# Bai-YT/ConsistencyTTA

Measured on AMD Instinct MI355X. Metric: 10s_audio_clips_per_sec_1step_gen, higher is better.
Workload: dtype bf16; 1 GPU; configs[1]: batch-32 single-step consistency inference, U-Net(light, 559M) + AudioLDM VAE decoder + HiFi-GAN, 10 s clips, L=32 text tokens, w=4, T5 excluded; batch_per_gpu=32, global_batch=32, text_len=32, waveform_samples=163872, weights=random-init (no checkpoints offline), parallelism=replicas x1 (clips sharded, no data-path collective)

## Files before the change

consistencytta_amd/_native.py:

```python
import ctypes
from ctypes import byref
import os
import subprocess
from ctypes import (POINTER, Structure, c_char_p, c_double, c_float, c_int, c_int16, c_int32,
                    c_int64, c_size_t, c_uint8, c_void_p)

_HERE = os.path.dirname(os.path.abspath(__file__))
LIB_PATH = os.path.join(_HERE, "libctta_hip.so")
CSRC = os.path.join(_HERE, "csrc")

MAX_LEVELS = 4
MAX_UPS = 8


class Tensor(Structure):
    _fields_ = [("name", c_char_p), ("data", c_void_p), ("ndim", c_int), ("shape", c_int64 * 4)]


class UNetConfig(Structure):
    _fields_ = [
        ("in_channels", c_int), ("out_channels", c_int), ("n_levels", c_int),
        ("block_out_channels", c_int * MAX_LEVELS), ("heads", c_int * MAX_LEVELS),
        ("layers_per_block", c_int * MAX_LEVELS), ("down_cross", c_int * MAX_LEVELS),
        ("up_cross", c_int * MAX_LEVELS), ("cross_attention_dim", c_int),
# ... 26 lines not shown
        ("n_kernels", c_int), ("upsample_rates", c_int * MAX_UPS),
        ("upsample_kernel_sizes", c_int * MAX_UPS), ("resblock_kernel_sizes", c_int * 4),
        ("resblock_dilations", (c_int * 3) * 4), ("max_batch", c_int), ("max_frames", c_int),
        ("debug_taps", c_int), ("enable_grad", c_int),
    ]


class FfnDesc(Structure):
    _fields_ = [("x", c_void_p), ("ld_x", c_int), ("M", c_int64), ("cp", c_int), ("ffp", c_int),
                ("packed", c_void_p), ("b1", c_void_p), ("b2", c_void_p), ("res", c_void_p), ("res_ld", c_int),
                ("out", c_void_p), ("ldc", c_int), ("n_valid", c_int),
                ("ln_gamma", c_void_p), ("ln_beta", c_void_p), ("ln_d", c_int), ("ln_eps", c_float),
                ("proj_packed", c_void_p), ("proj_bias", c_void_p), ("proj_res", c_void_p), ("proj_res_ld", c_int),
                ("front_packed", c_void_p), ("front_bias", c_void_p), ("att", c_void_p), ("att_ld", c_int), ("front_k", c_int),
                ("front_res", c_void_p), ("front_res_ld", c_int), ("s2_out", c_void_p), ("s2_ld", c_int)]


class ConvDesc(Structure):
    _fields_ = [
        ("x0", c_void_p), ("c0", c_int), ("x1", c_void_p), ("c1", c_int),
        ("batch", c_int), ("hi", c_int), ("wi", c_int), ("upsample", c_int),
        ("ho", c_int), ("wo", c_int),
        ("kh", c_int), ("kw", c_int), ("stride_h", c_int), ("stride_w", c_int),
        ("pad_h", c_int), ("pad_w", c_int), ("dil_h", c_int), ("dil_w", c_int),
        ("w", c_void_p), ("k_pad", c_int), ("n", c_int),
        ("bias", c_void_p), ("bias_m", c_void_p), ("rowvec", c_void_p), ("rowvec_ld", c_int),
        ("res", c_void_p), ("res_ld", c_int),
        ("in_act", c_int), ("in_slope", c_float), ("out_act", c_int), ("out_slope", c_float),
        ("alpha", c_float), ("accumulate", c_int), ("out", c_void_p), ("ldc", c_int), ("out_f32", c_int),
        ("out2", c_void_p), ("out2_slope", c_float),
# ... 136 lines not shown
    "ctta_wav_to_logmel_db_bwd": (c_int, [c_void_p, c_void_p, c_int, c_int, c_float, c_void_p, c_void_p]),
    "ctta_htsat_image": (c_int, [c_void_p, c_int, c_int, c_int, c_void_p, c_void_p, c_void_p, c_void_p, c_int, c_int, c_int,
                                 c_void_p, c_void_p]),
    "ctta_htsat_image_bwd": (c_int, [c_void_p, c_int, c_int, c_int, c_int, c_int, c_void_p, c_void_p, c_void_p, c_void_p,
                                     c_int, c_void_p, c_void_p]),
    "ctta_gather_rows": (c_int, [c_void_p, c_int, c_void_p, c_void_p, c_int, c_int64, c_int, c_void_p]),
    "ctta_gelu": (c_int, [c_void_p, c_void_p, c_int64, c_void_p]),
    "ctta_gelu_bwd": (c_int, [c_void_p, c_void_p, c_void_p, c_int64, c_void_p]),
    "ctta_mean_tokens": (c_int, [c_void_p, c_int, c_int, c_int, c_int, c_void_p, c_void_p]),
    "ctta_mean_tokens_bwd": (c_int, [c_void_p, c_int, c_int, c_int, c_int, c_void_p, c_void_p]),
    "ctta_resunit_supported": (c_int, [c_int, c_int, c_int]),
    "ctta_ffn_desc_init": (None, [c_void_p]),
    "ctta_ffn_proj_pack_bytes": (c_size_t, [c_int, c_int]),
    "ctta_ffn_proj_pack": (c_int, [c_void_p, c_int, c_int, c_int, c_void_p, c_void_p]),
    "ctta_ffn_block": (c_int, [c_void_p, c_void_p]),
    "ctta_ffn_geglu_supported": (c_int, [c_int, c_int]),
    "ctta_ffn_geglu_wanted": (c_int, [c_int, c_int, c_int64]),
    "ctta_ffn_pack_bytes": (c_size_t, [c_int, c_int]),
    "ctta_ffn_pack": (c_int, [c_void_p, c_int, c_void_p, c_int, c_int, c_int, c_void_p, c_void_p]),
    "ctta_ffn_geglu": (c_int, [c_void_p, c_int, c_int64, c_int, c_int, c_void_p, c_void_p, c_void_p, c_void_p, c_int, c_void_p,
                               c_int, c_int, c_void_p, c_void_p, c_int, c_float, c_void_p]),
    "ctta_frag_pack": (c_int, [c_void_p, c_int, c_int, c_int, c_void_p, c_void_p]),
    "ctta_resunit_conv1d": (c_int, [c_void_p, c_int, c_int, c_int, c_int, c_int, c_void_p, c_void_p, c_void_p, c_void_p,
                                    c_float, c_void_p, c_int, c_float, c_float, c_void_p]),
    "ctta_logmel_to_image": (c_int, [c_void_p, c_int, c_int, c_int, c_void_p, c_void_p, c_void_p, c_void_p]),
    "ctta_avgpool2": (c_int, [c_void_p, c_void_p, c_int, c_int, c_int, c_int, c_void_p]),
    "ctta_cnn14_head": (c_int, [c_void_p, c_int, c_int, c_int, c_int, c_void_p, c_void_p]),
    "ctta_reschain_supported": (c_int, [c_int, c_int, c_void_p]),
    "ctta_reschain_conv1d": (c_int, [c_void_p, c_int, c_int, c_int, c_int, c_void_p, c_void_p, c_void_p, c_void_p, c_void_p,
                                     c_float, c_void_p, c_int, c_float, c_float, c_void_p]),
# ... 143 lines not shown
```

consistencytta_amd/csrc/common.h:

```cpp
#pragma once
#include <hip/hip_runtime.h>
#include <stdint.h>
#include <stdio.h>
#include <string.h>

#include "../../include/ctta.h"

typedef uint16_t bf16_t;

typedef __attribute__((ext_vector_type(8))) __bf16 bf16x8_t;
typedef __attribute__((ext_vector_type(4))) float f32x4_t;

__device__ __forceinline__ float bf2f(bf16_t v) { return __uint_as_float(((uint32_t)v) << 16); }

typedef __attribute__((ext_vector_type(2))) __bf16 bf16x2_t;
typedef __attribute__((ext_vector_type(2))) float f32x2_t;
__device__ __forceinline__ bf16_t f2bf(float f) { return __builtin_bit_cast(bf16_t, (__bf16)f); }

__device__ __forceinline__ uint32_t pack2bf(float lo, float hi) {
  const f32x2_t v = {lo, hi};
  return __builtin_bit_cast(uint32_t, __builtin_convertvector(v, bf16x2_t));
}

__device__ __forceinline__ void unpack8(const uint4& v, float f[8]) {
// ... 48 lines not shown
template <int GL>
__device__ __forceinline__ float ln_group_sum(float v) {
  v = dpp_row_sum(v);
  {
    const unsigned u = __float_as_uint(v);
    const auto r = __builtin_amdgcn_permlane16_swap(u, u, false, false);
    v = __uint_as_float(r[0]) + __uint_as_float(r[1]);
  }
  if constexpr (GL == 64) {
    const unsigned u = __float_as_uint(v);
    const auto r = __builtin_amdgcn_permlane32_swap(u, u, false, false);
    v = __uint_as_float(r[0]) + __uint_as_float(r[1]);
  }
  return v;
}
__device__ __forceinline__ float wave_sum(float v) {
#pragma unroll
  for (int o = 32; o > 0; o >>= 1) v += __shfl_xor(v, o, 64);
  return v;
}
__device__ __forceinline__ float wave_max(float v) {
#pragma unroll
  for (int o = 32; o > 0; o >>= 1) v = fmaxf(v, __shfl_xor(v, o, 64));
  return v;
}

enum CttaOption {
  CTTA_OPT_XCD = 0,
  CTTA_OPT_SPLITK,
  CTTA_OPT_STREAMK,
  CTTA_OPT_STREAMK_GRID,
  CTTA_OPT_WGRAD_STREAM,
  CTTA_OPT_GN_FUSE,
  CTTA_OPT_FUSED_RES,
  CTTA_OPT_FFN_FUSE,
  CTTA_OPT_COUNT
};
extern int g_ctta_opt[CTTA_OPT_COUNT];
int ctta_cu_count();
static inline int ctta_opt(CttaOption o) { return g_ctta_opt[o]; }
void ctta_set_error(const char* fmt, ...);
bool ctta_prof_active();
bool ctta_gn_fuse_on();
unsigned long long* ctta_debug_stamps_current();
void ctta_prof_begin(int kind, int variant, long long m, long long n, long long k, long long groups, hipStream_t s);
void ctta_prof_end(hipStream_t s);
hipError_t ctta_zero_async(void* ptr, size_t bytes, hipStream_t s);

#define CTTA_CHECK_HIP(expr)                                                         \
  do {                                                                               \
    hipError_t _e = (expr);                                                          \
    if (_e != hipSuccess) {                                                          \
      ctta_set_error("%s:%d: %s -> %s", __FILE__, __LINE__, #expr, hipGetErrorString(_e)); \
      return CTTA_ERR_HIP;                                                           \
    }                                                                                \
  } while (0)

#define CTTA_REQUIRE(cond, ...)                \
// ... 26 lines not shown
```

consistencytta_amd/csrc/engine_unet.hip:

```cpp
#include "engine_common.h"

#include <stdlib.h>

#include <math.h>

__global__ void add_silu_kernel(const float* __restrict__ a, const float* __restrict__ b,
                                float* __restrict__ out, float* __restrict__ sum_out, int n) {
  const int i = blockIdx.x * blockDim.x + threadIdx.x;
  if (i >= n) return;
  const float v = a[i] + (b ? b[i] : 0.f);
  if (sum_out) sum_out[i] = v;
  out[i] = v / (1.0f + expf(-v));
}
__global__ void mask_bias_kernel(const uint8_t* __restrict__ m, float* __restrict__ out, int n) {
  const int i = blockIdx.x * blockDim.x + threadIdx.x;
  if (i < n) out[i] = (1.0f - (m[i] ? 1.0f : 0.0f)) * -10000.0f;
}
__global__ void pack_enc_kernel(const float* __restrict__ src, bf16_t* __restrict__ dst, int B, int L,
                                int X, int Lp, int Xp) {
  const long long total = (long long)B * Lp * Xp;
  for (long long i = blockIdx.x * (long long)blockDim.x + threadIdx.x; i < total;
       i += (long long)gridDim.x * blockDim.x) {
    const int x = (int)(i % Xp);
    const long long r = i / Xp;
// ... 26 lines not shown
  struct Saved { const bf16_t *x = nullptr, *a = nullptr, *t1 = nullptr, *a2 = nullptr; float *st1 = nullptr, *st2 = nullptr; int H = 0, W = 0; } sv;
};

struct LNLayer { float* gamma = nullptr; float* beta = nullptr; std::string key; };

struct Transformer {
  int c = 0, heads = 0, dh = 0, inner = 0, cp = 0, hp = 0, ffh = 0, ffp = 0;
  GNLayer norm;
  PackedW proj_in, qk1, v1, out1, q2, k2, v2, out2, ff1, ff2, proj_out;
  LNLayer ln1, ln2, ln3;
  bf16_t *k2c = nullptr, *vt2c = nullptr;
  bf16_t* ffn_stream = nullptr;
  bool want_proj_stream = false;
  bf16_t* front_stream = nullptr;
  bf16_t* proj_stream = nullptr;
  LinTrain t_proj_in, t_q1, t_k1, t_v1, t_out1, t_q2, t_k2, t_v2, t_out2, t_ff1, t_ff2, t_proj_out;
  struct Saved {
    const bf16_t *x = nullptr, *g = nullptr, *s0 = nullptr, *n1 = nullptr, *qk = nullptr, *vt = nullptr, *att1 = nullptr,
                 *s1 = nullptr, *n2 = nullptr, *q2 = nullptr, *k2 = nullptr, *vt2 = nullptr, *att2 = nullptr, *s2 = nullptr,
                 *n3 = nullptr, *f = nullptr, *gg = nullptr, *s3 = nullptr;
    float *st = nullptr, *lse1 = nullptr, *lse2 = nullptr;
    int H = 0, W = 0;
  } sv;
};

struct Level {
  std::vector<Resnet> res;
  std::vector<Transformer> att;
  bool has_sampler = false;
  ConvLayer sampler;
// ... 162 lines not shown
    ws.jobs.push_back([=](const WeightTable&, hipStream_t s) -> ctta_status { return ctta_ffn_pack(w1, k1, w2, k2, cp, ffp, dst, s); });
    T->want_proj_stream = true;
  }
  CTTA_TRY(make_ln(ws, t + "norm1.", inner, &T->ln1));
  CTTA_TRY(make_ln(ws, t + "norm2.", inner, &T->ln2));
  CTTA_TRY(make_ln(ws, t + "norm3.", inner, &T->ln3));
  CTTA_TRY(lin(p + "proj_out.weight", p + "proj_out.bias", c, inner, identity_map(c, round_up(c, 4)), in_cols,
               &T->proj_out, &T->t_proj_out));
  if (T->want_proj_stream && T->out2.n == cp && T->out2.k_pad == hp && T->out2.bias && ctta_ffn_proj_pack_bytes(cp, hp)) {
    T->front_stream = reinterpret_cast<bf16_t*>(ws.arena.get<unsigned char>(ctta_ffn_proj_pack_bytes(cp, hp)));
    if (!T->front_stream) { ctta_set_error("weight store exhausted (front projection weight stream)"); return CTTA_ERR_NOMEM; }
    const bf16_t* w0 = T->out2.w;
    bf16_t* dst = T->front_stream;
    ws.jobs.push_back([=](const WeightTable&, hipStream_t s) -> ctta_status { return ctta_ffn_proj_pack(w0, hp, hp, cp, dst, s); });
  }
  if (T->want_proj_stream && T->proj_out.n == cp && T->proj_out.k_pad == cp && c == cp) {
    T->proj_stream = reinterpret_cast<bf16_t*>(ws.arena.get<unsigned char>(ctta_ffn_proj_pack_bytes(cp, cp)));
    if (!T->proj_stream) { ctta_set_error("weight store exhausted (projection weight stream)"); return CTTA_ERR_NOMEM; }
    const bf16_t* w3 = T->proj_out.w;
    bf16_t* dst = T->proj_stream;
    ws.jobs.push_back([=](const WeightTable&, hipStream_t s) -> ctta_status { return ctta_ffn_proj_pack(w3, cp, cp, cp, dst, s); });
  }
  return CTTA_OK;
}

static ctta_status gn(UCtx& c, const GNLayer& g, const bf16_t* x, bf16_t* y, int hw, float eps, bool silu,
                      float** stats_out = nullptr) {
  const int groups = c.U->cfg.norm_num_groups;
  size_t need = ctta_groupnorm_scratch_floats(c.B, hw, g.c, groups);
  if (c.train) {
// ... 43 lines not shown
  }
  RUN(c, ctta_attention_lse(q, q_ld, k, k_ld, k_rows, vt, vt_ld, bias, out, out_ld, c.B, heads, nq, nk,
                            1.0f / sqrtf((float)dh), lse, c.stream));
  return CTTA_OK;
}

static ctta_status run_transformer(UCtx& c, Transformer& T, const bf16_t* x, int H, int W,
                                   bf16_t** out_p) {
  Arena& A = *c.arena;
  const int N = H * W;
  const size_t M = (size_t)c.B * N;
  const int cp = T.cp, hp = T.hp;
  bf16_t* out = A.get<bf16_t>(M * T.c); ALLOC_OR_FAIL(out);
  const size_t mk = A.mark();
  bf16_t* g = A.get<bf16_t>(M * T.c); ALLOC_OR_FAIL(g);
  CTTA_TRY(gn(c, T.norm, x, g, N, 1e-6f, false, &T.sv.st));
  bf16_t* s0 = A.get<bf16_t>(M * cp); ALLOC_OR_FAIL(s0);
  CTTA_TRY(run_linear(c, T.proj_in, g, T.c, M, s0, cp, nullptr, 0));
  bf16_t* n = A.get<bf16_t>(M * cp); ALLOC_OR_FAIL(n);
  RUN(c, ctta_layernorm(s0, n, M, T.inner, cp, T.ln1.gamma, T.ln1.beta, 1e-5f, c.stream));
  bf16_t* qk = A.get<bf16_t>(M * 2 * hp); ALLOC_OR_FAIL(qk);
  CTTA_TRY(run_linear(c, T.qk1, n, cp, M, qk, 2 * hp, nullptr, 0));
  const int vt_ld = round_up(N, 8);
  bf16_t* vt = A.get<bf16_t>((size_t)c.B * hp * vt_ld); ALLOC_OR_FAIL(vt);
  CTTA_TRY(run_vt(c, T.v1, n, c.B, N, N, vt, vt_ld));
  bf16_t* att = A.get<bf16_t>(M * hp); ALLOC_OR_FAIL(att);
  CTTA_TRY(run_attention(c, qk, 2 * hp, qk + hp, 2 * hp, N, vt, vt_ld, nullptr, att, hp, T.heads, N, N, T.dh, &T.sv.lse1));
  bf16_t* s1 = A.get<bf16_t>(M * cp); ALLOC_OR_FAIL(s1);
  CTTA_TRY(run_linear(c, T.out1, att, hp, M, s1, cp, s0, cp));
  bf16_t* const n1 = n;
  bf16_t* const att1 = att;
  if (c.train) {
    n = A.get<bf16_t>(M * cp); ALLOC_OR_FAIL(n);
    att = A.get<bf16_t>(M * hp); ALLOC_OR_FAIL(att);
  }
  RUN(c, ctta_layernorm(s1, n, M, T.inner, cp, T.ln2.gamma, T.ln2.beta, 1e-5f, c.stream));
  bf16_t* const n2 = n;
  bf16_t* q2 = A.get<bf16_t>(M * hp); ALLOC_OR_FAIL(q2);
  CTTA_TRY(run_linear(c, T.q2, n, cp, M, q2, hp, nullptr, 0));
  bf16_t* k2 = T.k2c;
  bf16_t* vt2 = T.vt2c;
  if (!k2 || c.dry) {
    k2 = A.get<bf16_t>((size_t)c.B * c.Lp * hp); ALLOC_OR_FAIL(k2);
    vt2 = A.get<bf16_t>((size_t)c.B * hp * c.Lp); ALLOC_OR_FAIL(vt2);
  }
  if (!c.reuse_text) {
    CTTA_TRY(run_linear(c, T.k2, c.enc_bf, c.U->xp, (int64_t)c.B * c.Lp, k2, hp, nullptr, 0));
    CTTA_TRY(run_vt(c, T.v2, c.enc_bf, c.B, c.Lp, c.Lp, vt2, c.Lp));
  }
  CTTA_TRY(run_attention(c, q2, hp, k2, hp, c.Lp, vt2, c.Lp, c.mask_bias, att, hp, T.heads, N, c.L, T.dh, &T.sv.lse2));
  bf16_t* s2 = A.get<bf16_t>(M * cp); ALLOC_OR_FAIL(s2);
  const bool ffn_fused = !c.train && T.ffn_stream && ctta_ffn_geglu_wanted(cp, T.ffp, (int64_t)M);
  const bool ffn_front = ffn_fused && T.front_stream;
  if (!ffn_front) {
    CTTA_TRY(run_linear(c, T.out2, att, hp, M, s2, cp, s1, cp));
    if (c.train) { n = A.get<bf16_t>(M * cp); ALLOC_OR_FAIL(n); }
    RUN(c, ctta_layernorm(s2, n, M, T.inner, cp, T.ln3.gamma, T.ln3.beta, 1e-5f, c.stream));
  }
  bf16_t* f = nullptr;
  bf16_t* gg = nullptr;
  if (c.train) {
    f = A.get<bf16_t>(M * 2 * T.ffp); ALLOC_OR_FAIL(f);
    CTTA_TRY(run_linear(c, T.ff1, n, cp, M, f, 2 * T.ffp, nullptr, 0));
    gg = A.get<bf16_t>(M * T.ffp); ALLOC_OR_FAIL(gg);
    RUN(c, ctta_geglu(f, gg, M, T.ffp, 1, c.stream));
  } else if (ffn_fused) {
    ctta_ffn_desc fd;
// ... 550 lines not shown
```

consistencytta_amd/csrc/norm_elem.hip:

```cpp
#include "common.h"

#include <math.h>
#include <stdlib.h>

__global__ void nchw_to_nhwc_kernel(const float* __restrict__ src, bf16_t* __restrict__ dst, int B,
                                    int C, int HW, int Cp, float scale) {
  const int vc = Cp / 8;
  const long long total = (long long)B * HW * vc;
  for (long long idx = blockIdx.x * (long long)blockDim.x + threadIdx.x; idx < total;
       idx += (long long)gridDim.x * blockDim.x) {
    const int v = (int)(idx % vc);
    const long long pix = idx / vc;
    const int b = (int)(pix / HW);
    const int hw = (int)(pix - (long long)b * HW);
    float f[8];
#pragma unroll
    for (int e = 0; e < 8; ++e) {
      const int c = v * 8 + e;
      f[e] = c < C ? src[((size_t)b * C + c) * HW + hw] * scale : 0.f;
    }
    *reinterpret_cast<uint4*>(dst + (size_t)pix * Cp + v * 8) = pack8(f);
  }
}

// ... 259 lines not shown
  __syncthreads();
  const int cpg = C / G;
  for (int g = tid; g < G; g += 256) {
    float s = 0.f, q = 0.f;
    for (int l = 0; l < PL; ++l)
      for (int cc = 0; cc < cpg; ++cc) {
        s += ssum[l * C + g * cpg + cc];
        q += ssq[l * C + g * cpg + cc];
      }
    float* o = part + (((size_t)b * nchunk + chunk) * G + g) * 2;
    o[0] = s;
    o[1] = q;
  }
}

__device__ __forceinline__ void gn_fold_chunks(const float* __restrict__ pg, int nchunk, int G, int l, int LPG, double& s,
                                               double& q) {
  constexpr int U = 8;
  for (int ch = l; ch < nchunk; ch += LPG * U) {
    float2 pp[U];
#pragma unroll
    for (int u = 0; u < U; ++u) {
      const int c = ch + u * LPG;
      pp[u] = c < nchunk ? *reinterpret_cast<const float2*>(pg + (size_t)c * G * 2) : make_float2(0.f, 0.f);
    }
#pragma unroll
    for (int u = 0; u < U; ++u) {
      s += (double)pp[u].x;
      q += (double)pp[u].y;
    }
  }
}

__global__ __launch_bounds__(256) void gn_finalize_kernel(const float* __restrict__ part, int nchunk, int G, int C,
                                                          int HW, const float* __restrict__ gamma,
                                                          const float* __restrict__ beta, float eps,
                                                          float* __restrict__ scale_shift, float* __restrict__ stats) {
  const int b = blockIdx.x;
  const int cpg = C / G;
  int LPG = 1;
  if (G <= 128 && 256 % G == 0) LPG = min(64, 256 / G);
  const int per_pass = 256 / LPG;
  for (int g0 = 0; g0 < G; g0 += per_pass) {
    const int g = g0 + (int)threadIdx.x / LPG, l = (int)threadIdx.x % LPG;
    double s = 0.0, q = 0.0;
    if (g < G) gn_fold_chunks(part + ((size_t)b * nchunk * G + g) * 2, nchunk, G, l, LPG, s, q);
    for (int off = 1; off < LPG; off <<= 1) {
// ... 828 lines not shown
```

include/ctta.h:

```cpp
#ifndef CTTA_H
#define CTTA_H

#include <stddef.h>
#include <stdint.h>

#ifdef __cplusplus
extern "C" {
#endif

typedef enum {
  CTTA_OK = 0,
  CTTA_ERR_INVALID = 1,
  CTTA_ERR_HIP = 2,
  CTTA_ERR_MISSING_KEY = 3,
  CTTA_ERR_NOMEM = 4
} ctta_status;

const char* ctta_last_error(void);
int ctta_version(void);

ctta_status ctta_set_option(const char* name, int value);
ctta_status ctta_get_option(const char* name, int* value);
int ctta_num_options(void);
const char* ctta_option_name(int i);
// ... 214 lines not shown
  int x_stride;
  void* gn_part; int gn_groups; int gn_hw;
  int64_t gn_part_floats;
} ctta_conv_desc;

ctta_status ctta_conv_gemm(const ctta_conv_desc* d, void* stream);
int ctta_conv_last_gn_chunks(void);
void ctta_conv_bind_workspace(void* ws, size_t bytes);
void ctta_conv_bind_workspace_ex(void* ws, size_t bytes, int header_zeroed);
int ctta_conv_bound_workspace_header(void);
size_t ctta_conv_workspace_header_bytes(void);
void ctta_conv_bound_workspace(void** ws, size_t* bytes);
void ctta_conv_suppress_splitk(int on);
void ctta_conv_debug_stamps(void* buf);
void ctta_attention_debug_stamps(void* buf);
size_t ctta_conv_workspace_bytes(void);
int ctta_conv_gemm_num_variants(void);
const char* ctta_conv_gemm_variant_name(int id);

int ctta_resunit_supported(int channels, int k, int dil);
ctta_status ctta_frag_pack(const void* packed, int n, int k_pad, int k_valid, void* dst, void* stream);
ctta_status ctta_resunit_conv1d(const void* x, int batch, int len, int channels, int k, int dil,
                                const void* w1_frag, const float* b1, const void* w2_frag, const float* b2,
                                float slope, void* out, int accumulate, float alpha, float out_slope, void* stream);
int ctta_reschain_supported(int channels, int k, const int* dils);
ctta_status ctta_reschain_conv1d(const void* x, int batch, int len, int channels, int k, const int* dils,
                                 const void* const* w1_frag, const float* const* b1, const void* const* w2_frag,
                                 const float* const* b2, float slope, void* out, int accumulate, float alpha,
                                 float out_slope, void* stream);

// ... 7 lines not shown
                           const float* ln_gamma, const float* ln_beta, int ln_d, float ln_eps, void* stream);
typedef struct {
  const void* x; int ld_x; int64_t M; int cp, ffp;
  const void* packed; const float* b1; const float* b2;
  const void* res; int res_ld;
  void* out; int ldc; int n_valid;
  const float* ln_gamma; const float* ln_beta; int ln_d; float ln_eps;
  const void* proj_packed; const float* proj_bias; const void* proj_res; int proj_res_ld;
  const void* front_packed; const float* front_bias; const void* att; int att_ld; int front_k;
  const void* front_res; int front_res_ld; void* s2_out; int s2_ld;
} ctta_ffn_desc;
void ctta_ffn_desc_init(ctta_ffn_desc* d);
size_t ctta_ffn_proj_pack_bytes(int cp, int k);
ctta_status ctta_ffn_proj_pack(const void* w_packed, int k_pad, int k, int cp, void* dst, void* stream);
ctta_status ctta_ffn_block(const ctta_ffn_desc* d, void* stream);

ctta_status ctta_conv_small_n(const void* x, int c, int batch, int hi, int wi, int kh, int kw,
                              int pad_h, int pad_w, const float* w, const float* bias, int n,
                              int in_act, float in_slope, int out_act, float* out_nchw,
                              void* out_bf16_nhwc, void* stream);

ctta_status ctta_pack_weight(const float* src, const int32_t* row_off, const int32_t* col_off,
                             const int32_t* row_aux, const int32_t* col_aux, int aux_limit,
                             int n_rows, int k_pad, void* dst, void* stream);

#define CTTA_PACK_ELEMS_PER_BLOCK 2048
#define CTTA_COPY_ELEMS_PER_BLOCK 16384
typedef struct {
  const float* src;
  const int32_t *row_off, *col_off, *row_aux, *col_aux;
// ... 218 lines not shown
```

Measured before the change: 436.3 clips/s.

## Fuse GroupNorm, proj_in, LayerNorm and QKV projections into one attention-head kernel

Adds a single kernel that finalizes GroupNorm statistics from the existing partial sums and applies GN to a row tile held in shared memory. The same kernel then runs proj_in with bias (also writing s0), applies LayerNorm in place, and computes the QK projection and the transposed V projection from weights prepacked per wave. It replaces a GN launch, two linear layers, a layernorm and a V-transpose GEMM, cutting launches and global round trips of intermediates. It only engages for cp 256/512 when the tile grid fills the device and GN partials are ready; otherwise the old path runs. Costs are extra packed-weight memory and a large hand-written kernel.

```diff
diff --git a/consistencytta_amd/_native.py b/consistencytta_amd/_native.py
--- a/consistencytta_amd/_native.py
+++ b/consistencytta_amd/_native.py
@@ -64,6 +64,14 @@
                 ("proj_packed", c_void_p), ("proj_bias", c_void_p), ("proj_res", c_void_p), ("proj_res_ld", c_int),
                 ("front_packed", c_void_p), ("front_bias", c_void_p), ("att", c_void_p), ("att_ld", c_int), ("front_k", c_int),
                 ("front_res", c_void_p), ("front_res_ld", c_int), ("s2_out", c_void_p), ("s2_ld", c_int)]
+
+
+class AttnHeadDesc(Structure):
+    _fields_ = [("x", c_void_p), ("x_ld", c_int), ("batch", c_int), ("tokens", c_int), ("c", c_int), ("cp", c_int), ("hp", c_int),
+                ("rows", c_int), ("gn_table", c_void_p), ("gn_partials", c_void_p), ("gn_nchunk", c_int), ("gn_groups", c_int),
+                ("gn_gamma", c_void_p), ("gn_beta", c_void_p), ("gn_eps", c_float), ("packed", c_void_p), ("b_in", c_void_p),
+                ("s0", c_void_p), ("s0_ld", c_int), ("ln_gamma", c_void_p), ("ln_beta", c_void_p), ("ln_d", c_int),
+                ("ln_eps", c_float), ("qk", c_void_p), ("qk_ld", c_int), ("vt", c_void_p), ("vt_ld", c_int)]
 
 
 class ConvDesc(Structure):
@@ -230,6 +238,13 @@
     "ctta_ffn_proj_pack_bytes": (c_size_t, [c_int, c_int]),
     "ctta_ffn_proj_pack": (c_int, [c_void_p, c_int, c_int, c_int, c_void_p, c_void_p]),
     "ctta_ffn_block": (c_int, [c_void_p, c_void_p]),
+    "ctta_attn_chain_debug_mode": (None, [c_int]),
+    "ctta_attn_head_desc_init": (None, [c_void_p]),
+    "ctta_attn_head_supported": (c_int, [c_int, c_int, c_int, c_int]),
+    "ctta_attn_head_wanted": (c_int, [c_int, c_int, c_int, c_int]),
+    "ctta_attn_head_pack_bytes": (c_size_t, [c_int, c_int]),
+    "ctta_attn_head_pack": (c_int, [c_void_p, c_int, c_void_p, c_int, c_void_p, c_int, c_int, c_int, c_void_p, c_void_p]),
+    "ctta_attn_head_chain": (c_int, [c_void_p, c_void_p]),
     "ctta_ffn_geglu_supported": (c_int, [c_int, c_int]),
     "ctta_ffn_geglu_wanted": (c_int, [c_int, c_int, c_int64]),
     "ctta_ffn_pack_bytes": (c_size_t, [c_int, c_int]),
diff --git a/consistencytta_amd/csrc/attn_chain.hip b/consistencytta_amd/csrc/attn_chain.hip
--- /dev/null
+++ b/consistencytta_amd/csrc/attn_chain.hip
@@ -0,0 +1,404 @@
+#include "conv_epilogue.h"
+
+#include <string.h>
+
+#include <type_traits>
+
+typedef unsigned u32x2_t __attribute__((ext_vector_type(2)));
+typedef unsigned u32x4_t __attribute__((ext_vector_type(4)));
+
+#ifndef CTTA_ATTN_CHAIN
+#define CTTA_ATTN_CHAIN 1
+#endif
+
+constexpr int AC_NW = 8;
+constexpr int AC_PF = 2;
+constexpr int HEAD_ROWS_256 = 128, HEAD_ROWS_512 = 64;
+
+struct HeadParams {
+  const bf16_t* x; int x_ld;
+  const float* table;
+  const float* part; int nchunk, G;
+  const float* gn_gamma; const float* gn_beta; float gn_eps;
+  int tokens;
+  const bf16_t* win; const float* bin;
+  bf16_t* s0; int s0_ld;
+  const float* ln_gamma; const float* ln_beta; int ln_d; float ln_eps;
+  const bf16_t* wqk; bf16_t* qk; int qk_ld;
+  const bf16_t* wv; bf16_t* vt; int vt_ld, hp;
+  int M, batch;
+};
+
+template <int NC, int PB>
+__device__ __forceinline__ void ac_gemm(const uint4* wp, const bf16_t* base, const int rs, const int steps, const int lq, const int lg,
+                                        f32x4_t (&acc)[NC][PB]) {
+  constexpr int PF = NC > 2 ? 1 : AC_PF;
+  bf16x8_t r0[PF + 1][NC];
+#pragma unroll
+  for (int i = 0; i < NC; ++i)
+#pragma unroll
+    for (int j = 0; j < PB; ++j) acc[i][j] = (f32x4_t){0.f, 0.f, 0.f, 0.f};
+#pragma unroll
+  for (int s = 0; s < PF; ++s)
+#pragma unroll
+    for (int i = 0; i < NC; ++i) r0[s][i] = __builtin_bit_cast(bf16x8_t, wp[(s * NC + i) * 64]);
+  wp += PF * NC * 64;
+  const bf16_t* bw = base + lq * rs + lg * 8;
+  for (int st = 0; st < steps; ++st) {
+#pragma unroll
+    for (int i = 0; i < NC; ++i) r0[PF][i] = __builtin_bit_cast(bf16x8_t, wp[(st * NC + i) * 64]);
+    __builtin_amdgcn_sched_barrier(0);
+#pragma unroll
+    for (int pb = 0; pb < PB; ++pb) {
+      const bf16x8_t bf = __builtin_bit_cast(bf16x8_t, *reinterpret_cast<const uint4*>(bw + pb * 16 * rs + st * 32));
+#pragma unroll
+      for (int i = 0; i < NC; ++i) acc[i][pb] = __builtin_amdgcn_mfma_f32_16x16x32_bf16(r0[0][i], bf, acc[i][pb], 0, 0, 0);
+    }
+#pragma unroll
+    for (int s = 0; s < PF; ++s)
+#pragma unroll
+      for (int i = 0; i < NC; ++i) r0[s][i] = r0[s + 1][i];
+  }
+}
+
+template <int CP, int BM>
+__device__ __forceinline__ void ac_layernorm_tile(bf16_t* atile, const int tid, const float* __restrict__ gamma, const float* __restrict__ beta,
+                                                  const int d, const float eps) {
+  constexpr int RS = CP + 8, CV = CP / 8, RPS = 512 / CV, NSW = BM / RPS;
+  const int cc = tid % CV, rr = tid / CV;
+  const float inv_d = 1.0f / (float)d;
+  float g[8], bt[8];
+#pragma unroll
+  for (int e = 0; e < 8; ++e) {
+    const int c = cc * 8 + e;
+    g[e] = c < d ? gamma[c] : 0.f;
+    bt[e] = c < d ? beta[c] : 0.f;
+  }
+#pragma unroll
+  for (int u = 0; u < NSW; ++u) {
+    float f[8];
+    unpack8(*reinterpret_cast<const uint4*>(atile + (rr + u * RPS) * RS + cc * 8), f);
+    float sum = 0.f;
+#pragma unroll
+    for (int e = 0; e < 8; ++e) {
+      if (cc * 8 + e >= d) f[e] = 0.f;
+      sum += f[e];
+    }
+    const float mean = ln_group_sum<CV>(sum) * inv_d;
+    float q = 0.f;
+#pragma unroll
+    for (int e = 0; e < 8; ++e)
+      if (cc * 8 + e < d) { const float t = f[e] - mean; q += t * t; }
+    const float rstd = rsqrtf(ln_group_sum<CV>(q) * inv_d + eps);
+    float o8[8];
+#pragma unroll
+    for (int e = 0; e < 8; ++e) o8[e] = cc * 8 + e < d ? (f[e] - mean) * rstd * g[e] + bt[e] : 0.f;
+    *reinterpret_cast<uint4*>(atile + (rr + u * RPS) * RS + cc * 8) = pack8(o8);
+  }
+}
+
+template <int S, int PB, bool VT>
+__device__ __forceinline__ void ac_col_passes(const uint4* wq, const bf16_t* tile, const int rs, bf16_t* out, const int ldc, const int n_out,
+                                              const size_t out_bytes, const int row0_off, const int w, const int lane) {
+  const int lq = lane & 15, lg = lane >> 4;
+  const __amdgpu_buffer_rsrc_t rso = __builtin_amdgcn_make_buffer_rsrc((void*)out, 0, (unsigned)out_bytes, 0x00020000);
+  const int ngroups = (n_out + 127) / 128;
+  auto pass = [&](auto nc_tag, const int col) {
+    constexpr int NC = decltype(nc_tag)::value;
+    const uint4* wp = wq + (size_t)w * (S + AC_PF) * NC * 64 + lane;
+    bf16x8_t r0[AC_PF + 1][NC];
+    f32x4_t acc[NC][PB];
+#pragma unroll
+    for (int i = 0; i < NC; ++i)
+#pragma unroll
+      for (int j = 0; j < PB; ++j) acc[i][j] = (f32x4_t){0.f, 0.f, 0.f, 0.f};
+#pragma unroll
+    for (int s = 0; s < AC_PF; ++s)
+#pragma unroll
+      for (int i = 0; i < NC; ++i) r0[s][i] = __builtin_bit_cast(bf16x8_t, wp[(s * NC + i) * 64]);
+    wp += AC_PF * NC * 64;
+    const bf16_t* bw = tile + lq * rs + lg * 8;
+#pragma unroll
+    for (int st = 0; st < S; ++st) {
+#pragma unroll
+      for (int i = 0; i < NC; ++i) r0[AC_PF][i] = __builtin_bit_cast(bf16x8_t, wp[(st * NC + i) * 64]);
+      __builtin_amdgcn_sched_barrier(0);
+#pragma unroll
+      for (int pb = 0; pb < PB; ++pb) {
+        const bf16x8_t bf = __builtin_bit_cast(bf16x8_t, *reinterpret_cast<const uint4*>(bw + pb * 16 * rs + st * 32));
+#pragma unroll
+        for (int i = 0; i < NC; ++i)
+          acc[i][pb] = VT ? __builtin_amdgcn_mfma_f32_16x16x32_bf16(bf, r0[0][i], acc[i][pb], 0, 0, 0)
+                          : __builtin_amdgcn_mfma_f32_16x16x32_bf16(r0[0][i], bf, acc[i][pb], 0, 0, 0);
+      }
+#pragma unroll
+      for (int s = 0; s < AC_PF; ++s)
+#pragma unroll
+        for (int i = 0; i < NC; ++i) r0[s][i] = r0[s + 1][i];
+    }
+#pragma unroll
+    for (int i = 0; i < NC; ++i) {
+      const int blk = col + (w * NC + i) * 16;
+      const bool live = blk < n_out;
+      const int vo = !live ? (int)0x80000000 : VT ? row0_off + ((blk + lq) * ldc + lg * 4) * 2 : row0_off + (lq * ldc + blk + lg * 4) * 2;
+#pragma unroll
+      for (int pb = 0; pb < PB; ++pb) {
+        const f32x4_t a = acc[i][pb];
+        u32x2_t pk;
+        pk[0] = pack2bf(a[0], a[1]);
+        pk[1] = pack2bf(a[2], a[3]);
+        __builtin_amdgcn_raw_buffer_store_b64(pk, rso, vo + (VT ? pb * 16 * 2 : pb * 16 * ldc * 2), 0, 0);
+      }
+    }
+  };
+  int col = 0;
+  for (int gp = 0; gp + 2 <= ngroups; gp += 2) {
+    pass(std::integral_constant<int, 2>{}, col);
+    wq += (size_t)AC_NW * (S + AC_PF) * 2 * 64;
+    col += 256;
+  }
+  if (ngroups & 1) pass(std::integral_constant<int, 1>{}, col);
+}
+
+
+template <int CP, int BM>
+__global__ __launch_bounds__(512, 4) void attn_head_kernel(const HeadParams p) {
+  constexpr int RS = CP + 8, S1 = CP / 32, NC2 = CP / 16 / AC_NW, PB = BM / 16;
+  constexpr int CV = CP / 8, RPS = 512 / CV, NSW = BM / RPS;
+  extern __shared__ __attribute__((aligned(16))) unsigned char smem_raw[];
+  bf16_t* atile = reinterpret_cast<bf16_t*>(smem_raw);
+  float* ss = reinterpret_cast<float*>(smem_raw + (size_t)BM * RS * 2);
+  const int tid = threadIdx.x, lane = tid & 63, w = __builtin_amdgcn_readfirstlane(tid >> 6);
+  const int lq = lane & 15, lg = lane >> 4;
+  const int m0 = blockIdx.x * BM, b = m0 / p.tokens;
+
+  {
+    const int cc = tid % CV, rr = tid / CV;
+    const __amdgpu_buffer_rsrc_t rsx =
+        __builtin_amdgcn_make_buffer_rsrc((void*)p.x, 0, (unsigned)((size_t)p.M * p.x_ld * 2), 0x00020000);
+    u32x4_t v[NSW];
+#pragma unroll
+    for (int u = 0; u < NSW; ++u) v[u] = __builtin_amdgcn_raw_buffer_load_b128(rsx, ((m0 + rr + u * RPS) * p.x_ld + cc * 8) * 2, 0, 0);
+    const float* tab = p.table ? p.table + (size_t)b * 2 * CP : ss;
+    if (!p.table) {
+      if (tid < 256) {
+        const int G = p.G, nchunk = p.nchunk, cpg = CP / G;
+        int LPG = 1;
+        if (G <= 128 && 256 % G == 0) LPG = min(64, 256 / G);
+        const int per_pass = 256 / LPG;
+        for (int g0 = 0; g0 < G; g0 += per_pass) {
+          const int g = g0 + tid / LPG, l = tid % LPG;
+          double s = 0.0, q = 0.0;
+          if (g < G) gn_fold_chunks(p.part + ((size_t)b * nchunk * G + g) * 2, nchunk, G, l, LPG, s, q);
+          for (int off = 1; off < LPG; off <<= 1) {
+            s += __shfl_xor(s, off);
+            q += __shfl_xor(q, off);
+          }
+          if (g >= G) continue;
+          const double n = (double)p.tokens * cpg;
+          const double mean = s / n;
+          double var = q / n - mean * mean;
+          if (var < 0.0) var = 0.0;
+          const float rstd = (float)(1.0 / sqrt(var + (double)p.gn_eps));
+          const float meanf = (float)mean;
+          for (int c2 = l; c2 < cpg; c2 += LPG) {
+            const int c = g * cpg + c2;
+            const float sc = rstd * p.gn_gamma[c];
+            ss[c] = sc;
+            ss[CP + c] = p.gn_beta[c] - meanf * sc;
+          }
+        }
+      }
+      __syncthreads();
+    }
+    float scl[8], shf[8];
+#pragma unroll
+    for (int e = 0; e < 8; ++e) { scl[e] = tab[cc * 8 + e]; shf[e] = tab[CP + cc * 8 + e]; }
+#pragma unroll
+    for (int u = 0; u < NSW; ++u) {
+      float f[8];
+      unpack8(make_uint4(v[u][0], v[u][1], v[u][2], v[u][3]), f);
+#pragma unroll
+      for (int e = 0; e < 8; ++e) f[e] = f[e] * scl[e] + shf[e];
+      *reinterpret_cast<uint4*>(atile + (rr + u * RPS) * RS + cc * 8) = pack8(f);
+    }
+  }
+  __syncthreads();
+
+  {
+    f32x4_t acc[NC2][PB];
+    ac_gemm<NC2, PB>(reinterpret_cast<const uint4*>(p.win) + (size_t)w * (S1 + AC_PF) * NC2 * 64 + lane, atile, RS, S1, lq, lg, acc);
+    __syncthreads();
+    const __amdgpu_buffer_rsrc_t rso =
+        __builtin_amdgcn_make_buffer_rsrc((void*)p.s0, 0, (unsigned)((size_t)p.M * p.s0_ld * 2), 0x00020000);
+    const int n0 = w * NC2 * 16 + lg * 4;
+#pragma unroll
+    for (int i = 0; i < NC2; ++i) {
+      const int n = n0 + i * 16;
+      const float4 bb = *reinterpret_cast<const float4*>(p.bin + n);
+      const int vo = ((m0 + lq) * p.s0_ld + n) * 2;
+#pragma unroll
+      for (int pb = 0; pb < PB; ++pb) {
+        const f32x4_t a = acc[i][pb];
+        u32x2_t pk;
+        pk[0] = pack2bf(a[0] + bb.x, a[1] + bb.y);
+        pk[1] = pack2bf(a[2] + bb.z, a[3] + bb.w);
+        *reinterpret_cast<u32x2_t*>(atile + (pb * 16 + lq) * RS + n) = pk;
+        __builtin_amdgcn_raw_buffer_store_b64(pk, rso, vo + pb * 16 * p.s0_ld * 2, 0, 0);
+      }
+    }
+  }
+  __syncthreads();
+
+  ac_layernorm_tile<CP, BM>(atile, tid, p.ln_gamma, p.ln_beta, p.ln_d, p.ln_eps);
+  __syncthreads();
+
+  ac_col_passes<S1, PB, false>(reinterpret_cast<const uint4*>(p.wqk), atile, RS, p.qk, p.qk_ld, 2 * p.hp, (size_t)p.M * p.qk_ld * 2,
+                               m0 * p.qk_ld * 2, w, lane);
+  ac_col_passes<S1, PB, true>(reinterpret_cast<const uint4*>(p.wv), atile, RS, p.vt, p.vt_ld, p.hp, (size_t)p.batch * p.hp * p.vt_ld * 2,
+                              (b * p.hp * p.vt_ld + (m0 - b * p.tokens)) * 2, w, lane);
+}
+
+__global__ void ac_pack_rows_kernel(const bf16_t* __restrict__ wsrc, int k_pad, int k, int cp, bf16_t* __restrict__ dst) {
+  const int S = k / 32, NC2 = cp / 16 / AC_NW;
+  const long long per = (long long)(S + AC_PF) * NC2 * 64, total = AC_NW * per;
+  for (long long t = blockIdx.x * (long long)blockDim.x + threadIdx.x; t < total; t += (long long)gridDim.x * blockDim.x) {
+    const int wv = (int)(t / per);
+    const long long r = t - wv * per;
+    const int lane = (int)(r & 63);
+    const long long f = r >> 6;
+    const int i = (int)(f % NC2), st = (int)(f / NC2);
+    uint4 v = make_uint4(0, 0, 0, 0);
+    if (st < S) v = *reinterpret_cast<const uint4*>(wsrc + (size_t)((wv * NC2 + i) * 16 + (lane & 15)) * k_pad + st * 32 + (lane >> 4) * 8);
+    reinterpret_cast<uint4*>(dst)[t] = v;
+  }
+}
+__global__ void ac_pack_cols_kernel(const bf16_t* __restrict__ wsrc, int k_pad, int n_out, int cp, bf16_t* __restrict__ dst) {
+  const int S1 = cp / 32, G = (n_out + 127) / 128;
+  const long long per2 = (long long)(S1 + AC_PF) * 2 * 64, per1 = (long long)(S1 + AC_PF) * 64;
+  const long long tot2 = (long long)(G / 2) * AC_NW * per2, total = tot2 + (G & 1) * AC_NW * per1;
+  for (long long t = blockIdx.x * (long long)blockDim.x + threadIdx.x; t < total; t += (long long)gridDim.x * blockDim.x) {
+    int nc, col0;
+    long long r;
+    if (t < tot2) { nc = 2; col0 = (int)(t / (AC_NW * per2)) * 256; r = t % (AC_NW * per2); }
+    else { nc = 1; col0 = (G / 2) * 256; r = t - tot2; }
+    const long long per = nc == 2 ? per2 : per1;
+    const int wv = (int)(r / per);
+    r -= wv * per;
+    const int lane = (int)(r & 63);
+    const long long f = r >> 6;
+    const int i = (int)(f % nc), st = (int)(f / nc);
+    const int row = col0 + (wv * nc + i) * 16 + (lane & 15);
+    uint4 v = make_uint4(0, 0, 0, 0);
+    if (st < S1 && row < n_out) v = *reinterpret_cast<const uint4*>(wsrc + (size_t)row * k_pad + st * 32 + (lane >> 4) * 8);
+    reinterpret_cast<uint4*>(dst)[t] = v;
+  }
+}
+
+static bool ac_shape_ok(int cp, int hp) { return (cp == 256 || cp == 512) && hp >= 64 && hp % 64 == 0 && hp <= 1024; }
+static size_t ac_rows_uint4(int cp, int k) { return (size_t)AC_NW * (k / 32 + AC_PF) * (cp / 16 / AC_NW) * 64; }
+static size_t ac_cols_uint4(int cp, int n_out) {
+  const size_t G = (n_out + 127) / 128, S1 = cp / 32;
+  return (G / 2) * AC_NW * (S1 + AC_PF) * 2 * 64 + (G & 1) * AC_NW * (S1 + AC_PF) * 64;
+}
+static ctta_status ac_pack_rows(const void* w, int k_pad, int k, int cp, bf16_t* dst, hipStream_t s) {
+  hipLaunchKernelGGL(ac_pack_rows_kernel, dim3(256), dim3(256), 0, s, (const bf16_t*)w, k_pad, k, cp, dst);
+  CTTA_LAUNCH_CHECK();
+  return CTTA_OK;
+}
+static ctta_status ac_pack_cols(const void* w, int k_pad, int n_out, int cp, bf16_t* dst, hipStream_t s) {
+  hipLaunchKernelGGL(ac_pack_cols_kernel, dim3(256), dim3(256), 0, s, (const bf16_t*)w, k_pad, n_out, cp, dst);
+  CTTA_LAUNCH_CHECK();
+  return CTTA_OK;
+}
+static int ac_fill_ok(long long tiles) {
+  const long long slots = 2LL * ctta_cu_count(), rounds = (tiles + slots - 1) / slots;
+  if (rounds == 1) return tiles * 4 >= ctta_cu_count() ? 1 : 0;
+  return tiles * 10 >= rounds * slots * 6 ? 1 : 0;
+}
+
+static int g_attn_chain_mode = CTTA_ATTN_CHAIN ? 1 : 0;
+extern "C" void ctta_attn_chain_debug_mode(int mode) { g_attn_chain_mode = mode < 0 ? 0 : mode > 2 ? 2 : mode; }
+int ctta_attn_chain_mode() { return g_attn_chain_mode; }
+
+static int head_rows(int cp) { return cp == 256 ? HEAD_ROWS_256 : HEAD_ROWS_512; }
+static bool head_rows_ok(int cp, int bm) { return cp == 256 ? (bm == 64 || bm == 128) : (bm == 32 || bm == 64); }
+
+extern "C" int ctta_attn_head_supported(int c, int cp, int hp, int tokens) {
+  return c == cp && ac_shape_ok(cp, hp) && tokens > 0 && tokens % head_rows(cp) == 0 ? 1 : 0;
+}
+extern "C" int ctta_attn_head_wanted(int cp, int hp, int batch, int tokens) {
+  if (!ctta_attn_head_supported(cp, cp, hp, tokens) || batch < 1) return 0;
+  return ac_fill_ok((long long)batch * tokens / head_rows(cp));
+}
+extern "C" size_t ctta_attn_head_pack_bytes(int cp, int hp) {
+  if (!ac_shape_ok(cp, hp)) return 0;
+  return (ac_rows_uint4(cp, cp) + ac_cols_uint4(cp, 2 * hp) + ac_cols_uint4(cp, hp)) * 16;
+}
+extern "C" ctta_status ctta_attn_head_pack(const void* w_in, int k_pad_in, const void* w_qk, int k_pad_qk, const void* w_v, int k_pad_v, int cp,
+                                           int hp, void* dst, void* stream) {
+  CTTA_REQUIRE(w_in && w_qk && w_v && dst, "attn_head_pack: null pointer");
+  CTTA_REQUIRE(ac_shape_ok(cp, hp) && k_pad_in >= cp && k_pad_qk >= cp && k_pad_v >= cp && k_pad_in % 8 == 0 && k_pad_qk % 8 == 0 && k_pad_v % 8 == 0,
+               "attn_head_pack: cp=%d (256 or 512), hp=%d (a multiple of 64, <= 1024), k_pad %d / %d / %d >= cp", cp, hp, k_pad_in, k_pad_qk, k_pad_v);
+  bf16_t* d0 = (bf16_t*)dst;
+  bf16_t* d1 = d0 + ac_rows_uint4(cp, cp) * 8;
+  bf16_t* d2 = d1 + ac_cols_uint4(cp, 2 * hp) * 8;
+  CTTA_TRY(ac_pack_rows(w_in, k_pad_in, cp, cp, d0, (hipStream_t)stream));
+  CTTA_TRY(ac_pack_cols(w_qk, k_pad_qk, 2 * hp, cp, d1, (hipStream_t)stream));
+  return ac_pack_cols(w_v, k_pad_v, hp, cp, d2, (hipStream_t)stream);
+}
+
+template <int CP, int BM>
+static ctta_status launch_head(const HeadParams& p, hipStream_t s) {
+  const size_t smem = (size_t)BM * (CP + 8) * 2 + (size_t)2 * CP * sizeof(float);
+  static bool configured = false;
+  if (!configured) {
+    CTTA_CHECK_HIP(hipFuncSetAttribute(reinterpret_cast<const void*>(&attn_head_kernel<CP, BM>),
+                                       hipFuncAttributeMaxDynamicSharedMemorySize, (int)smem));
+    configured = true;
+  }
+  attn_head_kernel<CP, BM><<<dim3((unsigned)(p.M / BM)), dim3(512), smem, s>>>(p);
+  return CTTA_OK;
+}
+
+extern "C" void ctta_attn_head_desc_init(ctta_attn_head_desc* d) { memset(d, 0, sizeof(*d)); }
+
+extern "C" ctta_status ctta_attn_head_chain(const ctta_attn_head_desc* d, void* stream) {
+  CTTA_REQUIRE(d, "attn_head_chain: null descriptor");
+  const int c = d->c, cp = d->cp, hp = d->hp, batch = d->batch, tokens = d->tokens;
+  CTTA_REQUIRE(d->x && d->packed && d->b_in && d->ln_gamma && d->ln_beta && d->s0 && d->qk && d->vt, "attn_head_chain: null pointer");
+  CTTA_REQUIRE(c == cp && ac_shape_ok(cp, hp), "attn_head_chain: c=%d cp=%d hp=%d is outside the chain's range (c == cp, 256 or 512; hp a multiple "
+               "of 64, <= 1024)", c, cp, hp);
+  const int bm = d->rows ? d->rows : head_rows(cp);
+  CTTA_REQUIRE(head_rows_ok(cp, bm), "attn_head_chain: no %d-row tile at cp=%d", bm, cp);
+  CTTA_REQUIRE(batch >= 1 && tokens >= 1 && tokens % bm == 0, "attn_head_chain: tokens=%d per sample is not a multiple of the %d-row tile", tokens, bm);
+  CTTA_REQUIRE(d->gn_table || (d->gn_partials && d->gn_gamma && d->gn_beta && d->gn_nchunk >= 1 && d->gn_groups >= 1 && cp % d->gn_groups == 0 &&
+                               (long long)d->gn_nchunk * d->gn_groups <= 2048),
+               "attn_head_chain: GroupNorm needs its scale / shift table, or partials (nchunk=%d x groups=%d <= 2048, groups dividing cp) with "
+               "gamma and beta", d->gn_nchunk, d->gn_groups);
+  const long long M = (long long)batch * tokens;
+  CTTA_REQUIRE(d->ln_d > 0 && d->ln_d <= cp && d->x_ld >= cp && d->x_ld % 8 == 0 && d->s0_ld >= cp && d->s0_ld % 4 == 0 && d->qk_ld >= 2 * hp &&
+               d->qk_ld % 4 == 0 && d->vt_ld >= tokens && d->vt_ld % 4 == 0 && M * d->x_ld * 2 < 0x7FF00000LL && M * d->s0_ld * 2 < 0x7FF00000LL &&
+               M * d->qk_ld * 2 < 0x7FF00000LL && (long long)batch * hp * d->vt_ld * 2 < 0x7FF00000LL,
+               "attn_head_chain: bad extents (M=%lld x_ld=%d s0_ld=%d qk_ld=%d vt_ld=%d ln_d=%d)", M, d->x_ld, d->s0_ld, d->qk_ld, d->vt_ld, d->ln_d);
+  HeadParams p;
+  memset(&p, 0, sizeof(p));
+  p.x = (const bf16_t*)d->x; p.x_ld = d->x_ld; p.table = d->gn_table;
+  p.part = d->gn_partials; p.nchunk = d->gn_nchunk; p.G = d->gn_groups; p.gn_gamma = d->gn_gamma; p.gn_beta = d->gn_beta; p.gn_eps = d->gn_eps;
+  p.tokens = tokens;
+  p.win = (const bf16_t*)d->packed; p.bin = d->b_in; p.s0 = (bf16_t*)d->s0; p.s0_ld = d->s0_ld;
+  p.ln_gamma = d->ln_gamma; p.ln_beta = d->ln_beta; p.ln_d = d->ln_d; p.ln_eps = d->ln_eps;
+  p.wqk = p.win + ac_rows_uint4(cp, cp) * 8; p.qk = (bf16_t*)d->qk; p.qk_ld = d->qk_ld;
+  p.wv = p.wqk + ac_cols_uint4(cp, 2 * hp) * 8; p.vt = (bf16_t*)d->vt; p.vt_ld = d->vt_ld; p.hp = hp;
+  p.M = (int)M; p.batch = batch;
+  hipStream_t s = (hipStream_t)stream;
+  const bool prof = ctta_prof_active();
+  if (prof) ctta_prof_begin(0, 46, M, cp, (long long)cp + 3LL * hp, 1, s);
+  ctta_status st;
+  if (cp == 512) st = bm == 64 ? launch_head<512, 64>(p, s) : launch_head<512, 32>(p, s);
+  else st = bm == 128 ? launch_head<256, 128>(p, s) : launch_head<256, 64>(p, s);
+  if (prof) ctta_prof_end(s);
+  CTTA_TRY(st);
+  CTTA_LAUNCH_CHECK();
+  return CTTA_OK;
+}
diff --git a/consistencytta_amd/csrc/common.h b/consistencytta_amd/csrc/common.h
--- a/consistencytta_amd/csrc/common.h
+++ b/consistencytta_amd/csrc/common.h
@@ -86,6 +86,24 @@
   }
   return v;
 }
+__device__ __forceinline__ void gn_fold_chunks(const float* __restrict__ pg, int nchunk, int G, int l, int LPG, double& s,
+                                               double& q) {
+  constexpr int U = 8;
+  for (int ch = l; ch < nchunk; ch += LPG * U) {
+    float2 pp[U];
+#pragma unroll
+    for (int u = 0; u < U; ++u) {
+      const int c = ch + u * LPG;
+      pp[u] = c < nchunk ? *reinterpret_cast<const float2*>(pg + (size_t)c * G * 2) : make_float2(0.f, 0.f);
+    }
+#pragma unroll
+    for (int u = 0; u < U; ++u) {
+      s += (double)pp[u].x;
+      q += (double)pp[u].y;
+    }
+  }
+}
+
 __device__ __forceinline__ float wave_sum(float v) {
 #pragma unroll
   for (int o = 32; o > 0; o >>= 1) v += __shfl_xor(v, o, 64);
@@ -114,6 +132,7 @@
 void ctta_set_error(const char* fmt, ...);
 bool ctta_prof_active();
 bool ctta_gn_fuse_on();
+int ctta_attn_chain_mode();
 unsigned long long* ctta_debug_stamps_current();
 void ctta_prof_begin(int kind, int variant, long long m, long long n, long long k, long long groups, hipStream_t s);
 void ctta_prof_end(hipStream_t s);
diff --git a/consistencytta_amd/csrc/engine_unet.hip b/consistencytta_amd/csrc/engine_unet.hip
--- a/consistencytta_amd/csrc/engine_unet.hip
+++ b/consistencytta_amd/csrc/engine_unet.hip
@@ -64,6 +64,7 @@
   bool want_proj_stream = false;
   bf16_t* front_stream = nullptr;
   bf16_t* proj_stream = nullptr;
+  bf16_t* head_stream = nullptr;
   LinTrain t_proj_in, t_q1, t_k1, t_v1, t_out1, t_q2, t_k2, t_v2, t_out2, t_ff1, t_ff2, t_proj_out;
   struct Saved {
     const bf16_t *x = nullptr, *g = nullptr, *s0 = nullptr, *n1 = nullptr, *qk = nullptr, *vt = nullptr, *att1 = nullptr,
@@ -256,6 +257,15 @@
     bf16_t* dst = T->front_stream;
     ws.jobs.push_back([=](const WeightTable&, hipStream_t s) -> ctta_status { return ctta_ffn_proj_pack(w0, hp, hp, cp, dst, s); });
   }
+  if (c == cp && ctta_attn_head_pack_bytes(cp, hp) && T->proj_in.n == cp && T->proj_in.k_pad >= cp && T->proj_in.bias && T->qk1.n == 2 * hp &&
+      T->qk1.k_pad >= cp && T->v1.n == hp && T->v1.k_pad >= cp) {
+    T->head_stream = reinterpret_cast<bf16_t*>(ws.arena.get<unsigned char>(ctta_attn_head_pack_bytes(cp, hp)));
+    if (!T->head_stream) { ctta_set_error("weight store exhausted (head chain weight streams)"); return CTTA_ERR_NOMEM; }
+    const bf16_t *wi = T->proj_in.w, *wqk = T->qk1.w, *wv = T->v1.w;
+    const int ki = T->proj_in.k_pad, kqk = T->qk1.k_pad, kv = T->v1.k_pad;
+    bf16_t* dst = T->head_stream;
+    ws.jobs.push_back([=](const WeightTable&, hipStream_t s) -> ctta_status { return ctta_attn_head_pack(wi, ki, wqk, kqk, wv, kv, cp, hp, dst, s); });
+  }
   if (T->want_proj_stream && T->proj_out.n == cp && T->proj_out.k_pad == cp && c == cp) {
     T->proj_stream = reinterpret_cast<bf16_t*>(ws.arena.get<unsigned char>(ctta_ffn_proj_pack_bytes(cp, cp)));
     if (!T->proj_stream) { ctta_set_error("weight store exhausted (projection weight stream)"); return CTTA_ERR_NOMEM; }
@@ -329,16 +339,35 @@
   bf16_t* out = A.get<bf16_t>(M * T.c); ALLOC_OR_FAIL(out);
   const size_t mk = A.mark();
   bf16_t* g = A.get<bf16_t>(M * T.c); ALLOC_OR_FAIL(g);
-  CTTA_TRY(gn(c, T.norm, x, g, N, 1e-6f, false, &T.sv.st));
   bf16_t* s0 = A.get<bf16_t>(M * cp); ALLOC_OR_FAIL(s0);
-  CTTA_TRY(run_linear(c, T.proj_in, g, T.c, M, s0, cp, nullptr, 0));
   bf16_t* n = A.get<bf16_t>(M * cp); ALLOC_OR_FAIL(n);
-  RUN(c, ctta_layernorm(s0, n, M, T.inner, cp, T.ln1.gamma, T.ln1.beta, 1e-5f, c.stream));
   bf16_t* qk = A.get<bf16_t>(M * 2 * hp); ALLOC_OR_FAIL(qk);
-  CTTA_TRY(run_linear(c, T.qk1, n, cp, M, qk, 2 * hp, nullptr, 0));
   const int vt_ld = round_up(N, 8);
   bf16_t* vt = A.get<bf16_t>((size_t)c.B * hp * vt_ld); ALLOC_OR_FAIL(vt);
-  CTTA_TRY(run_vt(c, T.v1, n, c.B, N, N, vt, vt_ld));
+  const int chain_mode = c.train || c.dry ? 0 : ctta_attn_chain_mode();
+  const bool head_chain = chain_mode > 0 && T.head_stream && ctta_attn_head_supported(T.c, cp, hp, N) &&
+                          (chain_mode == 2 || ctta_attn_head_wanted(cp, hp, c.B, N)) && c.gn_fpart && c.gn_ready_x == (const void*)x &&
+                          c.gn_ready_chunks > 0 && c.gn_ready_c == T.c && c.U->cfg.norm_num_groups == c.gn_groups &&
+                          (long long)c.gn_ready_chunks * c.gn_groups <= 2048;
+  if (head_chain) {
+    ctta_attn_head_desc hd;
+    ctta_attn_head_desc_init(&hd);
+    hd.x = x; hd.x_ld = T.c; hd.batch = c.B; hd.tokens = N; hd.c = T.c; hd.cp = cp; hd.hp = hp;
+    hd.gn_partials = c.gn_fpart; hd.gn_nchunk = c.gn_ready_chunks; hd.gn_groups = c.gn_groups;
+    hd.gn_gamma = T.norm.gamma; hd.gn_beta = T.norm.beta; hd.gn_eps = 1e-6f;
+    hd.packed = T.head_stream; hd.b_in = T.proj_in.bias; hd.s0 = s0; hd.s0_ld = cp;
+    hd.ln_gamma = T.ln1.gamma; hd.ln_beta = T.ln1.beta; hd.ln_d = T.inner; hd.ln_eps = 1e-5f;
+    hd.qk = qk; hd.qk_ld = 2 * hp; hd.vt = vt; hd.vt_ld = vt_ld;
+    c.gn_ready_x = nullptr;
+    c.gn_ready_chunks = 0;
+    RUN(c, ctta_attn_head_chain(&hd, c.stream));
+  } else {
+    CTTA_TRY(gn(c, T.norm, x, g, N, 1e-6f, false, &T.sv.st));
+    CTTA_TRY(run_linear(c, T.proj_in, g, T.c, M, s0, cp, nullptr, 0));
+    RUN(c, ctta_layernorm(s0, n, M, T.inner, cp, T.ln1.gamma, T.ln1.beta, 1e-5f, c.stream));
+    CTTA_TRY(run_linear(c, T.qk1, n, cp, M, qk, 2 * hp, nullptr, 0));
+    CTTA_TRY(run_vt(c, T.v1, n, c.B, N, N, vt, vt_ld));
+  }
   bf16_t* att = A.get<bf16_t>(M * hp); ALLOC_OR_FAIL(att);
   CTTA_TRY(run_attention(c, qk, 2 * hp, qk + hp, 2 * hp, N, vt, vt_ld, nullptr, att, hp, T.heads, N, N, T.dh, &T.sv.lse1));
   bf16_t* s1 = A.get<bf16_t>(M * cp); ALLOC_OR_FAIL(s1);
@@ -365,7 +394,7 @@
   }
   CTTA_TRY(run_attention(c, q2, hp, k2, hp, c.Lp, vt2, c.Lp, c.mask_bias, att, hp, T.heads, N, c.L, T.dh, &T.sv.lse2));
   bf16_t* s2 = A.get<bf16_t>(M * cp); ALLOC_OR_FAIL(s2);
-  const bool ffn_fused = !c.train && T.ffn_stream && ctta_ffn_geglu_wanted(cp, T.ffp, (int64_t)M);
+  const bool ffn_fused = !c.train && !c.dry && T.ffn_stream && ctta_ffn_geglu_wanted(cp, T.ffp, (int64_t)M);
   const bool ffn_front = ffn_fused && T.front_stream;
   if (!ffn_front) {
     CTTA_TRY(run_linear(c, T.out2, att, hp, M, s2, cp, s1, cp));
diff --git a/consistencytta_amd/csrc/norm_elem.hip b/consistencytta_amd/csrc/norm_elem.hip
--- a/consistencytta_amd/csrc/norm_elem.hip
+++ b/consistencytta_amd/csrc/norm_elem.hip
@@ -297,23 +297,6 @@
   }
 }
 
-__device__ __forceinline__ void gn_fold_chunks(const float* __restrict__ pg, int nchunk, int G, int l, int LPG, double& s,
-                                               double& q) {
-  constexpr int U = 8;
-  for (int ch = l; ch < nchunk; ch += LPG * U) {
-    float2 pp[U];
-#pragma unroll
-    for (int u = 0; u < U; ++u) {
-      const int c = ch + u * LPG;
-      pp[u] = c < nchunk ? *reinterpret_cast<const float2*>(pg + (size_t)c * G * 2) : make_float2(0.f, 0.f);
-    }
-#pragma unroll
-    for (int u = 0; u < U; ++u) {
-      s += (double)pp[u].x;
-      q += (double)pp[u].y;
-    }
-  }
-}
 
 __global__ __launch_bounds__(256) void gn_finalize_kernel(const float* __restrict__ part, int nchunk, int G, int C,
                                                           int HW, const float* __restrict__ gamma,
diff --git a/include/ctta.h b/include/ctta.h
--- a/include/ctta.h
+++ b/include/ctta.h
@@ -252,6 +252,7 @@
 void ctta_conv_suppress_splitk(int on);
 void ctta_conv_debug_stamps(void* buf);
 void ctta_attention_debug_stamps(void* buf);
+void ctta_attn_chain_debug_mode(int mode);
 size_t ctta_conv_workspace_bytes(void);
 int ctta_conv_gemm_num_variants(void);
 const char* ctta_conv_gemm_variant_name(int id);
@@ -289,6 +290,24 @@
 size_t ctta_ffn_proj_pack_bytes(int cp, int k);
 ctta_status ctta_ffn_proj_pack(const void* w_packed, int k_pad, int k, int cp, void* dst, void* stream);
 ctta_status ctta_ffn_block(const ctta_ffn_desc* d, void* stream);
+
+typedef struct {
+  const void* x; int x_ld; int batch, tokens, c, cp, hp, rows;
+  const float* gn_table; const float* gn_partials; int gn_nchunk, gn_groups;
+  const float* gn_gamma; const float* gn_beta; float gn_eps;
+  const void* packed; const float* b_in;
+  void* s0; int s0_ld;
+  const float* ln_gamma; const float* ln_beta; int ln_d; float ln_eps;
+  void* qk; int qk_ld;
+  void* vt; int vt_ld;
+} ctta_attn_head_desc;
+void ctta_attn_head_desc_init(ctta_attn_head_desc* d);
+int ctta_attn_head_supported(int c, int cp, int hp, int tokens);
+int ctta_attn_head_wanted(int cp, int hp, int batch, int tokens);
+size_t ctta_attn_head_pack_bytes(int cp, int hp);
+ctta_status ctta_attn_head_pack(const void* w_in, int k_pad_in, const void* w_qk, int k_pad_qk, const void* w_v, int k_pad_v, int cp,
+                                int hp, void* dst, void* stream);
+ctta_status ctta_attn_head_chain(const ctta_attn_head_desc* d, void* stream);
 
 ctta_status ctta_conv_small_n(const void* x, int c, int batch, int hi, int wi, int kh, int kw,
                               int pad_h, int pad_w, const float* w, const float* bias, int n,
```

Result: no change. 438.9 clips/s, median of 6 (+0.6%).
